# zoongahn/jodalroB-twoTower

Hardware: AMD Instinct MI355X
Metric: training pairs/sec at batch 8192 (embedding-lookup HBM GB/s in roofline) (higher is better)
Workload: dtype bf16 MFMA operands, f32 accumulate; f32 tables, master weights and activations (the tower input x, which the GEMMs round to bf16 anyway, is stored bf16)

## Files before the change

### jodalrob-twotower_amd/csrc/tt_gemm.h

```cpp
#pragma once
#include "tt_common.h"

struct GemmNT {
  const float* A; int64_t lda; const float* W; int64_t ldw; const float* bias; float* C; int64_t ldc;
  int64_t M, N, K; bool relu; float alpha; bool bf16 = false;
  void* workspace = nullptr; size_t workspace_bytes = 0;
  bool a_bf16 = false, c_bf16 = false;
  struct NtDeferred* defer = nullptr;
};
struct NtDeferred { const float* slabs; int64_t slab_stride; int splits; };
size_t tt_gemm_nt_workspace_bytes(int64_t M, int64_t N, int64_t K);
int tt_gemm_nt_batched(hipStream_t st, const GemmNT* items, int n);
int tt_gemm_nt(hipStream_t st, const float* A, int64_t lda, const float* W, int64_t ldw, const float* bias, float* C,
               int64_t ldc, int64_t M, int64_t N, int64_t K, bool relu, float alpha = 1.f);

struct GemmNN {
  const float* A; int64_t lda; const float* W; int64_t ldw; float* C; int64_t ldc; int64_t M, N, K; bool bf16 = false;
  bool c_bf16 = false;
};
int tt_gemm_nn_batched(hipStream_t st, const GemmNN* items, int n);

size_t tt_gemm_tn_workspace_bytes(int64_t M, int64_t N, int64_t R);
struct GemmTN {
  const float* A; int64_t lda; const float* B; int64_t ldb; float* C; int64_t ldc; int64_t M, N, R;
// ... 108 lines not shown

struct GemmBack {
  const float* dpre; int H;
  const void* x; int64_t ldx; int kx; bool x_bf16;
  const float* dense; int64_t ld_dense; int din;
  const float* w; int h0;
  float* dx; int64_t ld_dx; bool dx_bf16;
  float* dw; float* db; float* dwp; float* dbp;
  void* ws_dw; size_t ws_dw_bytes;
  void* ws_g; size_t ws_g_bytes;
  int64_t B;
  const void* w16 = nullptr;
};
bool tt_gemm_back_supported(const GemmBack* items, int n);
size_t tt_gemm_back_g_workspace_bytes(int64_t H, int64_t h0, int64_t din, int64_t B);
int tt_gemm_back_batched(hipStream_t st, const GemmBack* items, int n, TnPending* pending);
```

### jodalrob-twotower_amd/csrc/tt_gemm.hip

```cpp
#include "tt_gemm.h"

#include <stdlib.h>

namespace {

constexpr int BM = 64, BN = 64, BK = 16, PAD = 4, THREADS = 256;
using f32x16 = __attribute__((ext_vector_type(16))) float;

struct GemmArgs {
  const float* A; int64_t lda; const float* B; int64_t ldb; float* C; int64_t ldc; int64_t slab_stride;
  int M, N, K, kchunk, splits;
  const float* bias; int relu; float alpha; float* colsum_slab;
  int a_bf16 = 0, b_bf16 = 0, c_bf16 = 0;
  const float* proj_w = nullptr; int proj_ldw = 0, proj_h0 = 0;
};
struct GemmBatch { GemmArgs a[TT_MAX_SIDES]; };

template <int MODE, bool VEC>
struct TileLoader {
  float r[4];
  __device__ __forceinline__ void load(const float* __restrict__ P, int64_t ld, int x0, int X, int k0, int kend, int t) {
    if (MODE == 0) {
      const int row = t >> 2, kq = (t & 3) * 4;
      const int x = x0 + row, k = k0 + kq;
// ... 495 lines not shown
      const int m = m0 + wr * 32 + (r & 3) + 8 * (r >> 2) + 4 * lh;
      if (g.c_bf16) reinterpret_cast<uint16_t*>(g.C)[(int64_t)m * g.ldc + n] = tt_f2bf(acc[r]);
      else g.C[(int64_t)m * g.ldc + n] = acc[r];
    }
    __syncthreads();
  }
}

constexpr int kBackProbs = 3 * TT_MAX_SIDES;
struct BackBatch {
  GemmArgs g[kBackProbs];
  int role[kBackProbs], tiles_m[kBackProbs], tiles[kBackProbs], wg_end[kBackProbs];
  int n;
};

template <bool X_BF16>
__global__ __launch_bounds__(THREADS, 4) void gemm_back_kernel(BackBatch b) {
  int p = 0;
  while (p + 1 < b.n && (int)blockIdx.x >= b.wg_end[p]) ++p;
  const int local = (int)blockIdx.x - (p ? b.wg_end[p - 1] : 0);
  const int split = local / b.tiles[p], tile = local % b.tiles[p];
  const int bx = tile % b.tiles_m[p], by = tile / b.tiles_m[p];
  __shared__ __attribute__((aligned(16))) BackSmem sm;
  const GemmArgs& g = b.g[p];
  if (b.role[p] == 0) gemm_fast_tile<1, 1, true, false, X_BF16>(g, split, bx, by, sm);
  else if (b.role[p] == 1) gemm_fast_tile<1, 1, false, false, false, true>(g, split, bx, by, sm);
  else if (g.K == 64) {
    const int nt_cols = g.N / BN;
    if (g.b_bf16) gemm_nn_k64_tiles<true>(g, bx, by * kNnCols, min(kNnCols, nt_cols - by * kNnCols), sm);
    else gemm_nn_k64_tiles<false>(g, bx, by * kNnCols, min(kNnCols, nt_cols - by * kNnCols), sm);
  } else gemm_fast_tile<0, 1, false, false, false>(g, split, bx, by, sm);
}

__global__ __launch_bounds__(THREADS) void slab_reduce_kernel(SlabBatch batch) {
  slab_reduce_block(batch, (int)blockIdx.x, (int)gridDim.x, (int)blockIdx.y);
}

inline bool vec_ok(const float* p, int64_t ld, bool bf16_elems = false) {
// ... 232 lines not shown
  for (int i = 0; i < n; ++i) {
    const GemmBack& g = it[i];
    if (g.B < 64 || g.B % 64 || g.H < 64 || g.H % 64 || g.H > kProjMaxH || g.kx % 64 || g.h0 % 64 || g.h0 < 64 || g.h0 >= g.kx || g.din % 64) return false;
    if ((g.H / BM) * g.h0 > 256) return false;
    if (g.x_bf16 != it[0].x_bf16) return false;
    if (!tt_aligned(g.dpre, 16) || !tt_aligned(g.x, 16) || g.ldx % 8 || !tt_aligned(g.dense, 16) || g.ld_dense % 4 || !tt_aligned(g.w, 16) ||
        !tt_aligned(g.dx, 16) || g.ld_dx % 4)
      return false;
    if (!g.ws_dw || g.ws_dw_bytes < tt_gemm_tn_workspace_bytes(g.H, g.kx, g.B) || !g.ws_g ||
        g.ws_g_bytes < tt_gemm_back_g_workspace_bytes(g.H, g.h0, g.din, g.B))
      return false;
  }
  return true;
}

int tt_gemm_back_batched(hipStream_t st, const GemmBack* it, int n, TnPending* pending) {
  if (!pending || !tt_gemm_back_supported(it, n)) {
    tt_set_error("tt_gemm_back: unsupported shapes / missing pending queue");
    return TT_ERR_INVALID_ARG;
  }
  BackBatch b{};
  SlabArgs sa[3 * TT_MAX_SIDES];
  int ns = 0, wg = 0;
  int64_t maxtotal = 1;
  auto kchunk_of = [](int64_t R, int splits) { return (int)(tt_cdiv(tt_cdiv(R, splits), BK16) * BK16); };
  for (int role = 0; role < 3; ++role)
    for (int i = 0; i < n; ++i) {
      const GemmBack& g = it[i];
      const int s0 = tn_splits(g.H, g.kx, g.B), s1 = back_g_splits(g.H, g.din, g.B);
      float* slabs0 = reinterpret_cast<float*>((reinterpret_cast<uintptr_t>(g.ws_dw) + 255) & ~uintptr_t(255));
      float* cslab0 = slabs0 + (size_t)s0 * (size_t)g.H * (size_t)g.kx;
// ... 19 lines not shown
      } else {
        float* c = g.dx_bf16 ? reinterpret_cast<float*>(reinterpret_cast<uint16_t*>(g.dx) + g.h0) : g.dx + g.h0;
        const bool w16 = g.w16 != nullptr && g.H == 64 && tt_aligned(g.w16, 16);
        const float* wsrc = w16 ? reinterpret_cast<const float*>(reinterpret_cast<const uint16_t*>(g.w16) + g.h0) : g.w + g.h0;
        b.g[p] = GemmArgs{g.dpre, g.H, wsrc, g.kx, c, g.ld_dx, 0, (int)g.B, g.kx - g.h0, g.H, (int)(tt_cdiv(g.H, BK16) * BK16), 1,
                          nullptr, 0, 1.f, nullptr, 0, w16 ? 1 : 0, g.dx_bf16 ? 1 : 0};
        tm = (int)(g.B / BM); tn_ = (g.kx - g.h0) / BN;
        if (g.H == 64) tn_ = (int)tt_cdiv(tn_, kNnCols);
      }
      b.role[p] = role;
      b.tiles_m[p] = tm;
      b.tiles[p] = tm * tn_;
      wg += tm * tn_ * b.g[p].splits;
      b.wg_end[p] = wg;
    }
  if (it[0].x_bf16) gemm_back_kernel<true><<<wg, THREADS, 0, st>>>(b);
  else gemm_back_kernel<false><<<wg, THREADS, 0, st>>>(b);
  TT_LAUNCH_CHECK();
  if (pending->n + ns > kSlabItems)
    if (int rc = tt_gemm_tn_flush(st, pending)) return rc;
  for (int i = 0; i < ns; ++i) pending->sb.a[pending->n++] = sa[i];
  pending->maxtotal = maxtotal > pending->maxtotal ? maxtotal : pending->maxtotal;
  return TT_OK;
}

int tt_gemm_nt(hipStream_t st, const float* A, int64_t lda, const float* W, int64_t ldw, const float* bias, float* C,
               int64_t ldc, int64_t M, int64_t N, int64_t K, bool relu, float alpha) {
  GemmNT it{A, lda, W, ldw, bias, C, ldc, M, N, K, relu, alpha};
  return tt_gemm_nt_batched(st, &it, 1);
}
```

### jodalrob-twotower_amd/csrc/tt_riders.h

```cpp
#pragma once
#include "tt_common.h"

constexpr int kRiderThreads = 1024;
constexpr int kPlanLongSeg = 64;
struct PlanLong {
  int32_t* counters;
  int32_t* long_row; int32_t* long_base; int32_t* chunk_lo; int32_t* chunk_hi;
};
struct CompactRider {
  const int32_t* uniq_stage; const int32_t* seg_stage; const int32_t* ucount; const int32_t* ubase; const int32_t* uend;
  PlanLong pl;
  int n_keys; int64_t M;
  int32_t* unique_rows; int32_t* seg_offsets; int32_t* n_unique;
};
struct Finish2Rider {
  const float* part; int n_wg, Dp; float fb, unscale; float* out; float* loss_out;
};
struct BnFinishRider {
  const float* partial; int64_t pstride; int nchunks, H;
  float* mean; float* rstd; float* rm; float* rv; int64_t* nbt;
  float* out;
};
struct BnFinishRiders { BnFinishRider r[TT_MAX_SIDES]; };
constexpr int kBnFinStride = 2 * 64;
// ... 144 lines not shown
        pl.long_row[li] = before + u;
        pl.long_base[li] = cb;
        for (int32_t c = 0; c < nch; ++c) {
          pl.chunk_lo[cb + c] = s0 + c * kPlanLongSeg;
          pl.chunk_hi[cb + c] = min(s1, s0 + (c + 1) * kPlanLongSeg);
        }
      }
    }
  }
  if (ki == 0 && threadIdx.x == 0) {
    n_unique[0] = all;
    seg_offsets[all] = (int32_t)M;
  }
}

__device__ __forceinline__ void finish2_body(const Finish2Rider& fr) {
  const float* __restrict__ part = fr.part;
  const int n_wg = fr.n_wg, Dp = fr.Dp;
  const float fb = fr.fb, unscale = fr.unscale;
  float* __restrict__ out = fr.out;
  float* __restrict__ loss_out = fr.loss_out;

  __shared__ float red[4][4 + 2 * 256];
  __shared__ float prod[256];
  const int t = threadIdx.x, q = t >> 8, j0 = t & 255, stride = 4 + 2 * Dp;
  for (int j = j0; j < stride; j += 256) {
    float s = 0.f;
    for (int w0 = q; w0 < n_wg; w0 += 32) {
      float v[8];
#pragma unroll
      for (int k = 0; k < 8; ++k) v[k] = w0 + 4 * k < n_wg ? part[(int64_t)(w0 + 4 * k) * stride + j] : 0.f;
#pragma unroll
      for (int k = 0; k < 8; ++k) s += v[k];
    }
    red[q][j] = s;
  }
  __syncthreads();
  if (t < 256) {
    float p = 0.f;
    if (t < Dp) {
      const float u = (red[0][4 + t] + red[1][4 + t]) + (red[2][4 + t] + red[3][4 + t]);
      const float v = (red[0][4 + Dp + t] + red[1][4 + Dp + t]) + (red[2][4 + Dp + t] + red[3][4 + Dp + t]);
      p = u * v;
    }
    prod[t] = p;
  }
  __syncthreads();
  if (t < 64) {
    float p = (prod[t] + prod[t + 64]) + (prod[t + 128] + prod[t + 192]);
#pragma unroll
// ... 5 lines not shown
      const float dsum = (red[0][2] + red[1][2]) + (red[2][2] + red[3][2]);
      const float pos = dsum / fb;
      const float neg = (tot - dsum) / (fb * fb - fb);
      out[0] = 0.5f * l / fb;
      out[1] = hit / fb;
      out[2] = pos;
      out[3] = neg;
      out[4] = pos - neg;
      out[5] = 0.f;
      out[6] = tot;
      out[7] = 0.f;
      if (loss_out) loss_out[0] = out[0];
    }
  }
}
#endif
```

### jodalrob-twotower_amd/csrc/tt_score_bf16.hip

```cpp
#include "tt_score_bwd_parts.h"
#include "tt_tail_bwd.h"
#include "tt_deferred.h"

#include <stdlib.h>

namespace {

template <int KS, int AT>
__device__ __forceinline__ void mfma1(const bf16x8 (&bf)[KS], const bf16x8 (&ares)[AT][KS], f32x16 (&acc)[AT]) {
#pragma unroll
  for (int i = 0; i < AT; ++i)
#pragma unroll
    for (int r = 0; r < 16; ++r) acc[i][r] = 0.f;
#pragma unroll
  for (int s = 0; s < KS; ++s)
#pragma unroll
    for (int i = 0; i < AT; ++i) acc[i] = __builtin_amdgcn_mfma_f32_32x32x16_bf16(bf[s], ares[i][s], acc[i], 0, 0, 0);
}

template <int KS, int AT, bool X3>
__device__ __forceinline__ void mfma_s(const bf16x8 (&bh)[KS], const bf16x8 (&bl)[X3 ? KS : 1], const bf16x8 (&ah)[AT][KS],
                                       const bf16x8 (&al)[AT][X3 ? KS : 1], f32x16 (&acc)[AT]) {
  if constexpr (!X3) {
    mfma1<KS, AT>(bh, ah, acc);
// ... 448 lines not shown
          if (a < Ra && dd < args.D) dr.dA[(int64_t)a * args.D + dd] = dacc[i][d][r] * g;
        }
  }
}

template <bool TAIL>
struct TailHost {};
template <>
struct TailHost<true> { tttail::Batch<tttail::TailBwdArgs> batch; bool drop; float p; uint64_t seed0; const uint64_t* seed_dev; };

template <int KS, int AT, bool UNIT, bool LQ = false, bool TAIL = false>
__global__ __launch_bounds__(512) void score_bwd_tr_kernel(BwdArgs args, TailHost<TAIL> th) {
  constexpr int NW = 8, Dp = KS * 16, ROWS = 32 * AT, DT = KS / 2;
  constexpr int TLD = Dp + 8;
  constexpr int kRedB = (NW / 2) * ROWS * Dp * 4, kParkB = NW * 32 * TLD * 2;
  static_assert(!TAIL || (KS == 4 && AT == 2 && !LQ && tttail::kTailBwdLds + 64 * tttail::kTailTileLd * 4 <= kRedB + kParkB),
                "the tail's head and its d_emb tile lie over red | park of the <4, 2> form");
  __shared__ float red_s[TAIL ? 1 : (NW / 2) * ROWS * Dp];
  __shared__ __attribute__((aligned(16))) __bf16 park_s[TAIL ? 1 : NW][32 * TLD];
  __shared__ __attribute__((aligned(16))) char smem[TAIL ? kRedB + kParkB : 16];
  float* const red = TAIL ? reinterpret_cast<float*>(smem) : red_s;
  __bf16 (*const park)[32 * TLD] = TAIL ? reinterpret_cast<__bf16 (*)[32 * TLD]>(smem + kRedB) : park_s;
  using s16x4 = __attribute__((ext_vector_type(4))) short;
  using s16x8 = __attribute__((ext_vector_type(8))) short;
  const BwdSel dr = select_dir(args, blockIdx.y != 0);
  const float c1 = dr.c1, c2 = args.c2, kx = UNIT ? args.kexp : 1.f;
  const int Ra = dr.Ra, Rb = dr.Rb, off = dr.off;
  const float* const wt_b = dr.wt_b;
  const int a0 = (int)blockIdx.x * ROWS;
  if (a0 >= Ra) return;
  const int lane = threadIdx.x & 63, c = lane & 31, h = lane >> 5;
  const int wave = __builtin_amdgcn_readfirstlane(threadIdx.x >> 6);
  const int nT = (Rb + 31) / 32;
  bf16x8 ares[AT][KS];
  float ia[AT], ua[AT];
  int pos[AT];
#pragma unroll
  for (int i = 0; i < AT; ++i) {
    load_bfrag<KS>(dr.a_rows, a0 / 32 + i, c, h, ares[i]);
    a_row_setup<LQ>(dr, kx, a0 + 32 * i + c, ia[i], ua[i], pos[i]);
  }
  const int posmin = a0 + off, posmax = a0 + ROWS - 1 + off;
  f32x16 dacc[AT][DT];
  zero_acc(dacc);
  const bool have_inv = dr.inv_b != nullptr;
// ... 85 lines not shown
    }
  };
  Tile T0, T1;
  load(T0, min(wave, tlast));
  __builtin_amdgcn_sched_barrier(0);
  for (int t = wave; t < nT; t += 2 * NW) {
    load(T1, min(t + NW, tlast));
    compute(T0, t);
    load(T0, min(t + 2 * NW, tlast));
    if (t + NW < nT) compute(T1, t + NW);
  }
  [[maybe_unused]] tttail::TailBwdConst<512> hk;
  [[maybe_unused]] tttail::TailBwdRows<512> hv;
  [[maybe_unused]] uint64_t hseed = 0;
  if constexpr (TAIL) {
    const tttail::TailBwdArgs& f = th.batch.a[blockIdx.y];
    tttail::tail_bwd_load_const<512>(f, hk);
    tttail::tail_bwd_load_rows<512, true>(f, min(f.col.B, a0 + 64), a0, hv);
    if (th.drop) hseed = tttail::seed_of(th.seed0, th.seed_dev);
  }
#pragma unroll
  for (int half = NW / 2; half >= 1; half >>= 1) {
    if (wave >= half && wave < 2 * half) {
      float* slab = red + (wave - half) * ROWS * Dp;
#pragma unroll
      for (int i = 0; i < AT; ++i)
#pragma unroll
        for (int d = 0; d < DT; ++d)
#pragma unroll
          for (int r = 0; r < 16; ++r) slab[(32 * i + rowmap(r, h)) * Dp + 32 * d + c] = dacc[i][d][r];
    }
    __syncthreads();
    if (wave < half) {
      const float* slab = red + wave * ROWS * Dp;
#pragma unroll
      for (int i = 0; i < AT; ++i)
#pragma unroll
        for (int d = 0; d < DT; ++d)
#pragma unroll
          for (int r = 0; r < 16; ++r) dacc[i][d][r] += slab[(32 * i + rowmap(r, h)) * Dp + 32 * d + c];
    }
    __syncthreads();
  }
  [[maybe_unused]] float* const htile = reinterpret_cast<float*>(smem + tttail::kTailBwdLds);
  if (wave == 0) {
    const float g = args.d_loss[0] * dr.out_scale;
#pragma unroll
    for (int i = 0; i < AT; ++i)
#pragma unroll
      for (int d = 0; d < DT; ++d)
#pragma unroll
        for (int r = 0; r < 16; ++r) {
          const int a = a0 + 32 * i + rowmap(r, h);
          const int dd = 32 * d + c;
          if (a < Ra && dd < args.D) dr.dA[(int64_t)a * args.D + dd] = dacc[i][d][r] * g;
          if constexpr (TAIL) htile[(32 * i + rowmap(r, h)) * tttail::kTailTileLd + dd] = dacc[i][d][r] * g;
        }
  }
  if constexpr (TAIL) tttail::tail_bwd_head<512, true>(th.batch.a[blockIdx.y], blockIdx.x, th.drop, th.p, hseed, smem, htile, &hk, &hv);
}

template <int KS, bool UNIT, bool FP8, int AT, int NWV, bool LQ = false>
__global__ __launch_bounds__(NWV * 64) void score_bwd_rows_kernel(BwdArgs args) {
  constexpr int NTH = NWV * 64, DT = KS / 2, Dp = KS * 16, K64 = FP8 ? KS / 4 : 1;
  constexpr int kRowsB = FP8 ? KS * 512 : KS * 1024, kFragB = KS * 1024, kIvB = 256, kStageB = kRowsB + kFragB + kIvB;
  constexpr int kPieces = (kRowsB + kFragB) / 16, kPPT = (kPieces + NTH - 1) / NTH;
  static_assert(!FP8 || KS % 4 == 0, "fp8 operands come in K = 64 steps");
  constexpr bool ALDS = !FP8 && KS == 16;
  extern __shared__ __attribute__((aligned(16))) char lds_raw[];
  const bool d1 = blockIdx.y != 0;
  DirBwd dr;
  dr.a_rows = d1 ? args.d[1].a_rows : args.d[0].a_rows;
  dr.b_rows = d1 ? args.d[1].b_rows : args.d[0].b_rows;
  dr.b_frag = d1 ? args.d[1].b_frag : args.d[0].b_frag;
// ... 655 lines not shown
                        tt_stream stream) {
  return fwd_bf16(ctx, dirs, n_dirs, D, inv_t, shift, stream, true, "tt_score_fwd_bf16x3");
}

int tt_score_bwd_bf16x3(tt_ctx* ctx, const tt_score_bwd_dir* dirs, int32_t n_dirs, int32_t D, float inv_t, float shift,
                        const float* d_loss, float scale, tt_stream stream) {
  return bwd_bf16x3(ctx, dirs, nullptr, n_dirs, D, inv_t, shift, d_loss, scale, stream, "tt_score_bwd_bf16x3");
}

int tt_score_bwd_bf16x3_lq(tt_ctx* ctx, const tt_score_bwd_dir* dirs, const tt_score_bwd_lq* lq, int32_t n_dirs, int32_t D,
                           float inv_t, float shift, const float* d_loss, float scale, tt_stream stream) {
  TT_CHECK_ARG(lq, "tt_score_bwd_bf16x3_lq: NULL lq");
  return bwd_bf16x3(ctx, dirs, lq, n_dirs, D, inv_t, shift, d_loss, scale, stream, "tt_score_bwd_bf16x3_lq");
}

}
```

### jodalrob-twotower_amd/csrc/tt_tail_bwd.h

```cpp
#pragma once
#include "tt_common.h"

namespace tttail {

constexpr float kNormEps = 1e-12f;

__device__ __forceinline__ float dropout_scale(bool on, float p, uint64_t seed, uint64_t idx) {
  if (!on) return 1.f;
  return tt_uniform01(seed, idx) >= p ? 1.f / (1.f - p) : 0.f;
}
__device__ __forceinline__ uint64_t seed_of(uint64_t seed, const uint64_t* seed_dev) { return seed_dev ? seed + seed_dev[0] : seed; }

template <typename A>
struct Batch {
  A a[TT_MAX_SIDES];
};

struct ColArgs {
  const float* x; int64_t ldx;
  const float* pre; const float* mean; const float* rstd;
  uint64_t salt;
  int B, H, rows_per_chunk, nchunks;
  float* partial; float* out0; float* out1;
  int64_t pstride = 0;
// ... 8 lines not shown

using tl_f32x16 = __attribute__((ext_vector_type(16))) float;
using tl_bf16x8 = __attribute__((ext_vector_type(8))) __bf16;
constexpr int kTailLd = 72;
constexpr int kTailLdF = 65;

struct TailBwdArgs {
  const float* y; const float* emb; const float* d_emb; float* d_y; int D;
  const float* w_out; const float* act; float* d_act;
  ColArgs col;
  float* w_slab; float* b_slab;
};

constexpr int kTailBwdLds = 2 * (2 * 64 * kTailLd) + 2 * (64 * kTailLd) + 2 * (64 * kTailLd) + 4 * (64 * kTailLdF) + 4 * (3 * 4 * 64);
static_assert(sizeof(float) * 64 * kTailLdF <= sizeof(__bf16) * 2 * 64 * kTailLd, "XH must fit over dyA | dyT");
constexpr int kTailTileLd = 72;

template <int NT>
struct TailBwdConst {
  static constexpr int R = 64 * 64 / NT;
  float w[R], mean, rstd;
};
template <int NT>
struct TailBwdRows {
  static constexpr int R = 64 * 64 / NT;
  float yv[R], e[R], de[R], av[R], pr[R];
};

template <int NT>
__device__ __forceinline__ void tail_bwd_load_const(const TailBwdArgs& f, TailBwdConst<NT>& k) {
  constexpr int NWV = NT / 64, R = TailBwdConst<NT>::R;
  const int H = f.col.H, D = f.D;
  const int c = threadIdx.x & 63, rq = threadIdx.x >> 6;
#pragma unroll
  for (int j = 0; j < R; ++j) {
    const int d = rq + NWV * j;
    k.w[j] = f.w_out[(int64_t)min(d, D - 1) * H + min(c, H - 1)];
  }
  k.mean = c < H ? f.col.mean[c] : 0.f;
  k.rstd = c < H ? f.col.rstd[c] : 0.f;
}

template <int NT, bool TILE>
__device__ __forceinline__ void tail_bwd_load_rows(const TailBwdArgs& f, int r1, int b0, TailBwdRows<NT>& v) {
  constexpr int NWV = NT / 64, R = TailBwdRows<NT>::R;
  const int H = f.col.H, D = f.D;
  const int c = threadIdx.x & 63, rq = threadIdx.x >> 6;
  const int lane = c, wave = rq;
#pragma unroll
  for (int j = 0; j < R; ++j) {
    const int r = b0 + wave * R + j;
    const bool ok = r < r1 && lane < D;
    const int64_t i = (int64_t)min(r, r1 - 1) * D + min(lane, D - 1);
    const float v0 = f.y[i], v1 = f.emb[i];
    v.yv[j] = ok ? v0 : 0.f;
    v.e[j] = ok ? v1 : 0.f;
    if constexpr (!TILE) {
      const float v2 = f.d_emb[i];
      v.de[j] = ok ? v2 : 0.f;
    }
  }
#pragma unroll
  for (int j = 0; j < R; ++j) {
    const int r = b0 + rq + NWV * j;
    const bool ok = c < H && r < r1;
    const int64_t i = (int64_t)min(r, r1 - 1) * H + min(c, H - 1);
    const float v0 = f.act[i], v1 = f.col.pre[i];
    v.av[j] = ok ? v0 : 0.f;
    v.pr[j] = ok ? v1 : 0.f;
  }
}

template <int NT, bool TILE>
__device__ __forceinline__ void tail_bwd_head(const TailBwdArgs& f, int chunk, bool drop, float p, uint64_t seed, char* smem,
                                              const float* tile, const TailBwdConst<NT>* pk, const TailBwdRows<NT>* pv) {
  static_assert(NT == 1024 || NT == 512, "the ordered parts run in the first four waves; the rest splits 64 rows over NT / 64");
  constexpr int NWV = NT / 64, R = 64 * 64 / NT;
  const ColArgs& a = f.col;
  const int H = a.H, D = f.D;
  __bf16* dy2 = reinterpret_cast<__bf16*>(smem);
  __bf16* Wn = dy2 + 2 * 64 * kTailLd;
  __bf16* actT = Wn + 64 * kTailLd;
  float* DY = reinterpret_cast<float*>(actT + 64 * kTailLd);
  float (*sh)[4][64] = reinterpret_cast<float (*)[4][64]>(DY + 64 * kTailLdF);
  __bf16* dyA = dy2;
  __bf16* dyT = dy2 + 64 * kTailLd;
  float* XH = reinterpret_cast<float*>(dy2);
  const int t = threadIdx.x, c = t & 63, rq = t >> 6;
  const int lane = c, wave = rq;
  const int r0 = chunk * a.rows_per_chunk, r1 = min(a.B, r0 + a.rows_per_chunk);
  TailBwdConst<NT> k;
  if constexpr (TILE) k = *pk;
  else tail_bwd_load_const<NT>(f, k);
#pragma unroll
  for (int j = 0; j < R; ++j) {
    const int d = rq + NWV * j;
    Wn[c * kTailLd + d] = (__bf16)((d < D && c < H) ? k.w[j] : 0.f);
  }
  const float mean = k.mean, rstd = k.rstd;
  tl_f32x16 accw;
#pragma unroll
  for (int i = 0; i < 16; ++i) accw[i] = 0.f;
  float s0 = 0.f, s1 = 0.f, cs = 0.f;
  for (int b0 = r0; b0 < r1; b0 += 64) {
    TailBwdRows<NT> v;
    if constexpr (TILE) {
      v = *pv;
      __syncthreads();
#pragma unroll
      for (int j = 0; j < R; ++j) {
        const int row = wave * R + j;
        const float v2 = tile[row * kTailTileLd + lane];
        v.de[j] = (b0 + row < r1 && lane < D) ? v2 : 0.f;
      }
    } else {
      tail_bwd_load_rows<NT, false>(f, r1, b0, v);
    }
    float ss[R], dot[R], xh[R], sc[R];
#pragma unroll
    for (int j = 0; j < R; ++j) {
      ss[j] = mul_rn(v.yv[j], v.yv[j]);
      dot[j] = mul_rn(v.e[j], v.de[j]);
    }
#pragma unroll
    for (int o = 32; o > 0; o >>= 1) {
#pragma unroll
      for (int j = 0; j < R; ++j) {
        ss[j] += __shfl_xor(ss[j], o);
        dot[j] += __shfl_xor(dot[j], o);
// ... 7 lines not shown
      float out = nrm > kNormEps ? (v.de[j] - v.e[j] * dot[j]) / den : v.de[j] / den;
      if (r < r1 && lane < D) f.d_y[(int64_t)r * D + lane] = out;
      else out = 0.f;
      DY[row * kTailLdF + lane] = out;
      dyA[row * kTailLd + lane] = (__bf16)out;
      dyT[lane * kTailLd + row] = (__bf16)out;
    }
#pragma unroll
    for (int j = 0; j < R; ++j) {
      const int row = rq + NWV * j, r = b0 + row;
      actT[c * kTailLd + row] = (__bf16)v.av[j];
      xh[j] = (fmaxf(v.pr[j], 0.f) - mean) * rstd;
      sc[j] = (c < H && r < r1) ? dropout_scale(drop, p, seed, a.salt + (uint64_t)((int64_t)r * H + c)) : 0.f;
    }
    __syncthreads();
    const int wr = (wave >> 1) & 1, wc = wave & 1, li = lane & 31, lh = lane >> 5;
    tl_f32x16 acc;
#pragma unroll
    for (int i = 0; i < 16; ++i) acc[i] = 0.f;
    if (wave < 4) {
      if (c < D) {
#pragma unroll
        for (int j = 0; j < 16; ++j) cs += DY[(rq + 4 * j) * kTailLdF + c];
      }
#pragma unroll
      for (int s2 = 0; s2 < 4; ++s2) {
        const int ko = 16 * s2 + 8 * lh;
        const tl_bf16x8 a1 = *reinterpret_cast<const tl_bf16x8*>(dyA + (wr * 32 + li) * kTailLd + ko);
        const tl_bf16x8 b1 = *reinterpret_cast<const tl_bf16x8*>(Wn + (wc * 32 + li) * kTailLd + ko);
        acc = __builtin_amdgcn_mfma_f32_32x32x16_bf16(a1, b1, acc, 0, 0, 0);
        const tl_bf16x8 a2 = *reinterpret_cast<const tl_bf16x8*>(dyT + (wr * 32 + li) * kTailLd + ko);
        const tl_bf16x8 b2 = *reinterpret_cast<const tl_bf16x8*>(actT + (wc * 32 + li) * kTailLd + ko);
        accw = __builtin_amdgcn_mfma_f32_32x32x16_bf16(a2, b2, accw, 0, 0, 0);
      }
    }
    __syncthreads();
    if (wave < 4) {
      const int n = wc * 32 + li;
#pragma unroll
      for (int r = 0; r < 16; ++r) DY[(wr * 32 + (r & 3) + 8 * (r >> 2) + 4 * lh) * kTailLdF + n] = acc[r];
    }
    __syncthreads();
#pragma unroll
    for (int j = 0; j < R; ++j) {
      const int row = rq + NWV * j, r = b0 + row;
      const float da = DY[row * kTailLdF + c] * sc[j];
      if (c < H && r < r1) f.d_act[(int64_t)r * H + c] = da;
      DY[row * kTailLdF + c] = da;
      XH[row * kTailLdF + c] = xh[j];
    }
    __syncthreads();
    if (t < 256 && c < H) {
      const int nrow = min(64, r1 - b0);
      for (int row = rq; row < nrow; row += 4) {
        const float da = DY[row * kTailLdF + c];
        s0 += da;
        s1 += da * XH[row * kTailLdF + c];
      }
    }
    __syncthreads();
  }
  if (t < 256) {
    sh[0][rq][c] = s0;
    sh[1][rq][c] = s1;
    sh[2][rq][c] = cs;
  }
  __syncthreads();
  if (t < 64) {
    if (c < H) {
      float* q = a.partial + (int64_t)chunk * 2 * H;
      q[c] = ((sh[0][0][c] + sh[0][1][c]) + sh[0][2][c]) + sh[0][3][c];
      q[H + c] = ((sh[1][0][c] + sh[1][1][c]) + sh[1][2][c]) + sh[1][3][c];
    }
    if (c < D) f.b_slab[(int64_t)chunk * D + c] = ((sh[2][0][c] + sh[2][1][c]) + sh[2][2][c]) + sh[2][3][c];
  }
  if (wave < 4) {
    const int wr = wave >> 1, wc = wave & 1, li = lane & 31, lh = lane >> 5;
    float* ws = f.w_slab + (int64_t)chunk * D * H;
    const int n = wc * 32 + li;
#pragma unroll
    for (int r = 0; r < 16; ++r) {
      const int m = wr * 32 + (r & 3) + 8 * (r >> 2) + 4 * lh;
      if (m < D && n < H) ws[(int64_t)m * H + n] = accw[r];
    }
  }
}

}

int tt_score_tail_bwd_launch(tt_ctx* ctx, const tttail::Batch<tttail::TailBwdArgs>& tb, bool drop, float p, uint64_t seed,
                             const uint64_t* seed_dev);
```

### jodalrob-twotower_amd/csrc/tt_tower.hip

```cpp
#include "tt_deferred.h"
#include "tt_tail_bwd.h"

namespace {

using namespace tttail;

constexpr int kThreads = 256;

struct BnStatArgs {
  const float* pre; int B, H, rows_per_chunk, nchunks; float* partial; float* mean; float* rstd; float* rm; float* rv; int64_t* nbt;
  int64_t pstride = 0;
};

__global__ __launch_bounds__(kThreads) void bn_stats_partial_kernel(Batch<BnStatArgs> batch) {
  const BnStatArgs& a = batch.a[blockIdx.z];
  const int H = a.H;
  if ((int)blockIdx.x * 64 >= H || (int)blockIdx.y >= a.nchunks) return;
  __shared__ Wf sh[4][64];
  const int c = blockIdx.x * 64 + (threadIdx.x & 63), rl = threadIdx.x >> 6;
  const int r0 = blockIdx.y * a.rows_per_chunk, r1 = min(a.B, r0 + a.rows_per_chunk);
  Wf w{0.f, 0.f, 0.f};
  if (c < H && r0 + rl < r1) {
    const float x0 = fmaxf(a.pre[(int64_t)(r0 + rl) * H + c], 0.f);
    float s = 0.f, q = 0.f, cnt = 0.f;
// ... 914 lines not shown
      *reinterpret_cast<bf16x4*>(f.pk_frag + fi * 8 + (q >> 3) * 4) = o;
    }
  }
}

__global__ __launch_bounds__(kTailThreads) void tail_bwd_kernel(Batch<TailBwdArgs> batch, bool drop, float p, uint64_t seed0,
                                                               const uint64_t* __restrict__ seed_dev, Finish2Rider fr, int fr_on) {
  if (fr_on && blockIdx.y == 0) {
    if (blockIdx.x == 0) finish2_body(fr);
    return;
  }
  const TailBwdArgs& f = batch.a[blockIdx.y - fr_on];
  if ((int)blockIdx.x >= f.col.nchunks) return;
  __shared__ __attribute__((aligned(16))) char smem[kTailBwdLds];
  const uint64_t seed = drop ? seed_of(seed0, seed_dev) : 0;
  tail_bwd_head<kTailThreads, false>(f, blockIdx.x, drop, p, seed, smem, nullptr, nullptr, nullptr);
}

struct TailApplyArgs {
  ColArgs col; BnBwdArgs bn;
  const float* w_slab; const float* b_slab; int D; float* g_w_out; float* g_b_out;
  int slab_chunks;
  float out_scale;
};

__global__ __launch_bounds__(kTailThreads) void tail_bwd_apply_kernel(Batch<TailApplyArgs> batch, Finish2Rider fr, int fr_on) {
  if (fr_on && blockIdx.y == 0) {
    if (blockIdx.x == 0) finish2_body(fr);
    return;
  }
  const TailApplyArgs& ta = batch.a[blockIdx.y - fr_on];
// ... 714 lines not shown
    TT_LAUNCH_CHECK();
  }
  for (int t = 0; t < n; ++t) {
    const tt_tower_grads* g = G[t];
    const float* in_last = nh == 0 ? reinterpret_cast<const float*>(A[t]->x) : A[t]->act[nh - 1];
    const int lw = last_width(P[t]);
    tn[t] = GemmTN{g->d_y, P[t]->d_out, in_last, lw, g->w_out, lw, P[t]->d_out, lw, B, ws[t].tn[nh + 1], ws[t].tn_bytes[nh + 1], g->b_out};
    dcur[t] = nh == 0 ? reinterpret_cast<float*>(g->d_x) : g->scratch[nh - 1];
    TT_CHECK_ARG(dcur[t], "tt_towers_mlp_bwd: NULL scratch buffer");
    nn[t] = GemmNN{g->d_y, P[t]->d_out, P[t]->w_out, lw, dcur[t], lw, B, lw, P[t]->d_out};
    tn[t].b_bf16 = nh == 0 && P[t]->x_dtype == TT_BF16;
    nn[t].c_bf16 = nh == 0 && P[t]->dx_dtype == TT_BF16;
  }
  for (int t = 0; t < n; ++t) tn[t].bf16 = nn[t].bf16 = P[0]->compute_dtype == TT_BF16;
  TnPending pend;
  if (fused) {
    const int i = nh - 1;
    Batch<TailBwdArgs> tb{};
    Batch<TailApplyArgs> tp{};
    int cmax = 1;
    for (int t = 0; t < n; ++t) {
      const tt_tower_grads* g = G[t];
      const int H = P[t]->hidden[i], D = P[t]->d_out;
      TT_CHECK_ARG(g->w[i] && g->b[i] && g->bn_w[i] && g->bn_b[i], "tt_towers_mlp_bwd: NULL gradient buffers of block %d", i);
      const int nchunks = chunks_for(B, H);
      const uint64_t salt = (((uint64_t)(i + 1) << 40) ^ ((uint64_t)t << 52)) + (uint64_t)P[t]->rng_row_offset * (uint64_t)H;
      const ColArgs col{nullptr, 0, A[t]->pre[i], A[t]->mean[i], A[t]->rstd[i], salt, (int)B, H, (int)tt_cdiv(B, nchunks), nchunks,
                        ws[t].col, g->bn_b[i], g->bn_w[i]};
      float* w_slab = reinterpret_cast<float*>((reinterpret_cast<uintptr_t>(ws[t].tn[nh + 1]) + 255) & ~uintptr_t(255));
      float* b_slab = w_slab + (size_t)nchunks * D * H;
// ... 22 lines not shown
    const int fr_on = (mine & TT_DQ_LOSS) ? 1 : 0;
    if (phase != 2 && !hosted) {
      tail_bwd_kernel<<<dim3((unsigned)cmax, (unsigned)(n + fr_on)), kTailThreads, 0, st>>>(tb, drop, dropout_p, seed, seed_dev, ctx->dq->loss,
                                                                                           fr_on);
      tt_deferred_taken(ctx, TT_DQ_LOSS & mine);
      TT_LAUNCH_CHECK();
    }
    if (phase == 1) {
      Batch<LocalArgs> la{};
      for (int t = 0; t < n; ++t) la.a[t] = LocalArgs{tb.a[t].col.partial, tb.a[t].col.nchunks, tb.a[t].col.H, G[t]->s_sync_local};
      tail_local_colsum_kernel<<<dim3(1, (unsigned)n), kThreads, 0, st>>>(la);
      TT_LAUNCH_CHECK();
      return TT_OK;
    }
    {
      const int fr_here = hosted ? fr_on : 0;
      tail_bwd_apply_kernel<<<dim3((unsigned)tt_cdiv(B, 64), (unsigned)(n + fr_here)), kTailThreads, 0, st>>>(tp, ctx->dq->loss, fr_here);
      if (fr_here) tt_deferred_taken(ctx, TT_DQ_LOSS);
      TT_LAUNCH_CHECK();
    }
  } else if (wide) {
    const int i = nh - 1;
    if (phase != 2) {
      Batch<TailBwdArgs> tb{};
      int cmax = 1;
      for (int t = 0; t < n; ++t) {
        const int H = P[t]->hidden[i];
        const int nchunks = chunks_for(B, H);
        const uint64_t salt = (((uint64_t)(i + 1) << 40) ^ ((uint64_t)t << 52)) + (uint64_t)P[t]->rng_row_offset * (uint64_t)H;
        const ColArgs col{nullptr, 0, A[t]->pre[i], A[t]->mean[i], A[t]->rstd[i], salt, (int)B, H, (int)tt_cdiv(B, nchunks), nchunks,
                          ws[t].col, G[t]->bn_b[i], G[t]->bn_w[i]};
// ... 68 lines not shown
    for (int t = 0; t < n; ++t) {
      const tt_tower_grads* g = G[t];
      const int H = P[t]->hidden[i];
      const int iw = in_width(P[t], i);
      const float* in_i = i == 0 ? reinterpret_cast<const float*>(A[t]->x) : A[t]->act[i - 1];
      tn[t] = GemmTN{dcur[t], H, in_i, iw, g->w[i], iw, H, iw, B, ws[t].tn[1 + i], ws[t].tn_bytes[1 + i], g->b[i]};
      tn[t].b_bf16 = i == 0 && P[t]->x_dtype == TT_BF16;
      float* dnext = i == 0 ? reinterpret_cast<float*>(g->d_x) : g->scratch[i - 1];
      TT_CHECK_ARG(dnext, "tt_towers_mlp_bwd: NULL scratch buffer");
      nn[t] = GemmNN{dcur[t], H, P[t]->w[i], iw, dnext, iw, B, iw, H};
      nn[t].c_bf16 = i == 0 && P[t]->dx_dtype == TT_BF16;
      dcur[t] = dnext;
    }
    for (int t = 0; t < n; ++t) tn[t].bf16 = nn[t].bf16 = P[0]->compute_dtype == TT_BF16;
    if (i == 0 && P[0]->compute_dtype == TT_BF16) {
      GemmBack gb[TT_MAX_SIDES];
      bool ok = true;
      for (int t = 0; t < n; ++t) {
        const tt_tower_grads* g = G[t];
        const int wx = P[t]->h0 + P[t]->kcat_e;
        ok = ok && !(P[t]->flags & TT_TOWER_UNFUSED_BACK);
        gb[t] = GemmBack{tn[t].A, P[t]->hidden[0], A[t]->x, wx, wx, P[t]->x_dtype == TT_BF16, A[t]->dense, P[t]->din, P[t]->din,
                         P[t]->w[0], P[t]->h0, reinterpret_cast<float*>(g->d_x), wx, P[t]->dx_dtype == TT_BF16, g->w[0], g->b[0],
                         g->w_proj, g->b_proj, ws[t].tn[1], ws[t].tn_bytes[1], ws[t].tn[0], ws[t].tn_bytes[0], B};
        gb[t].w16 = P[t]->w_bf16[0];
      }
      if (ok && tt_gemm_back_supported(gb, n)) {
        if (int rc = tt_gemm_back_batched(st, gb, n, &pend)) return rc;
        if (ctx->dq->defer_slabs) return tt_deferred_queue_slabs(ctx, st, &pend);
        return tt_gemm_tn_flush(st, &pend);
      }
    }
    if (int rc = tt_gemm_tn_batched(st, tn, n, &pend)) return rc;
    if (int rc = tt_gemm_nn_batched(st, nn, n)) return rc;
  }
  for (int t = 0; t < n; ++t) {
    const tt_tower_grads* g = G[t];
    const int wx = P[t]->h0 + P[t]->kcat_e;
    tn[t] = GemmTN{reinterpret_cast<const float*>(g->d_x), wx, A[t]->dense, P[t]->din, g->w_proj, P[t]->din, P[t]->h0, P[t]->din, B,
                   ws[t].tn[0], ws[t].tn_bytes[0], g->b_proj};
    tn[t].a_bf16 = P[t]->dx_dtype == TT_BF16;
  }
  for (int t = 0; t < n; ++t) tn[t].bf16 = P[0]->compute_dtype == TT_BF16;
// ... 32 lines not shown
```

Before: 37.33 million.

## Move loss-finish rider into gemm_back and keep tail d_emb in registers

The deferred loss reduction (finish2) now rides as an extra workgroup of the fused backward GEMM kernel instead of the tail-apply kernel, reusing the GEMM's LDS. In the fused score-backward tail, the wave reduction is restructured into a single-level split-and-sum in which each thread reads its rows of d_emb straight into registers. This replaces the staged LDS tile and the extra sync inside tail_bwd_head. Optional timestamp probes are added behind a compile flag. This is meant to shorten the tail-apply critical path and cut LDS traffic, at the cost of more register pressure and a heavier first GEMM block.

```diff
diff --git a/jodalrob-twotower_amd/csrc/tt_gemm.h b/jodalrob-twotower_amd/csrc/tt_gemm.h
--- a/jodalrob-twotower_amd/csrc/tt_gemm.h
+++ b/jodalrob-twotower_amd/csrc/tt_gemm.h
@@ -1,5 +1,6 @@
 #pragma once
 #include "tt_common.h"
+#include "tt_riders.h"
 
 struct GemmNT {
   const float* A; int64_t lda; const float* W; int64_t ldw; const float* bias; float* C; int64_t ldc;
@@ -146,4 +147,4 @@
 };
 bool tt_gemm_back_supported(const GemmBack* items, int n);
 size_t tt_gemm_back_g_workspace_bytes(int64_t H, int64_t h0, int64_t din, int64_t B);
-int tt_gemm_back_batched(hipStream_t st, const GemmBack* items, int n, TnPending* pending);
+int tt_gemm_back_batched(hipStream_t st, const GemmBack* items, int n, TnPending* pending, const Finish2Rider* rider = nullptr);
diff --git a/jodalrob-twotower_amd/csrc/tt_gemm.hip b/jodalrob-twotower_amd/csrc/tt_gemm.hip
--- a/jodalrob-twotower_amd/csrc/tt_gemm.hip
+++ b/jodalrob-twotower_amd/csrc/tt_gemm.hip
@@ -533,14 +533,20 @@
   int n;
 };
 
+static_assert(sizeof(BackSmem) >= sizeof(float) * kFinish2Lds, "the loss reduction runs in the tiles' LDS");
 template <bool X_BF16>
-__global__ __launch_bounds__(THREADS, 4) void gemm_back_kernel(BackBatch b) {
+__global__ __launch_bounds__(THREADS, 4) void gemm_back_kernel(BackBatch b, Finish2Rider fr, int fr_on) {
+  __shared__ __attribute__((aligned(16))) BackSmem sm;
+  if (fr_on && blockIdx.x == 0) {
+    finish2_body<THREADS>(fr, reinterpret_cast<float*>(&sm));
+    return;
+  }
+  const int wg = (int)blockIdx.x - fr_on;
   int p = 0;
-  while (p + 1 < b.n && (int)blockIdx.x >= b.wg_end[p]) ++p;
-  const int local = (int)blockIdx.x - (p ? b.wg_end[p - 1] : 0);
+  while (p + 1 < b.n && wg >= b.wg_end[p]) ++p;
+  const int local = wg - (p ? b.wg_end[p - 1] : 0);
   const int split = local / b.tiles[p], tile = local % b.tiles[p];
   const int bx = tile % b.tiles_m[p], by = tile / b.tiles_m[p];
-  __shared__ __attribute__((aligned(16))) BackSmem sm;
   const GemmArgs& g = b.g[p];
   if (b.role[p] == 0) gemm_fast_tile<1, 1, true, false, X_BF16>(g, split, bx, by, sm);
   else if (b.role[p] == 1) gemm_fast_tile<1, 1, false, false, false, true>(g, split, bx, by, sm);
@@ -803,7 +809,7 @@
   return true;
 }
 
-int tt_gemm_back_batched(hipStream_t st, const GemmBack* it, int n, TnPending* pending) {
+int tt_gemm_back_batched(hipStream_t st, const GemmBack* it, int n, TnPending* pending, const Finish2Rider* rider) {
   if (!pending || !tt_gemm_back_supported(it, n)) {
     tt_set_error("tt_gemm_back: unsupported shapes / missing pending queue");
     return TT_ERR_INVALID_ARG;
@@ -853,8 +859,10 @@
       wg += tm * tn_ * b.g[p].splits;
       b.wg_end[p] = wg;
     }
-  if (it[0].x_bf16) gemm_back_kernel<true><<<wg, THREADS, 0, st>>>(b);
-  else gemm_back_kernel<false><<<wg, THREADS, 0, st>>>(b);
+  const int fr_on = rider ? 1 : 0;
+  const Finish2Rider fr = rider ? *rider : Finish2Rider{};
+  if (it[0].x_bf16) gemm_back_kernel<true><<<wg + fr_on, THREADS, 0, st>>>(b, fr, fr_on);
+  else gemm_back_kernel<false><<<wg + fr_on, THREADS, 0, st>>>(b, fr, fr_on);
   TT_LAUNCH_CHECK();
   if (pending->n + ns > kSlabItems)
     if (int rc = tt_gemm_tn_flush(st, pending)) return rc;
diff --git a/jodalrob-twotower_amd/csrc/tt_riders.h b/jodalrob-twotower_amd/csrc/tt_riders.h
--- a/jodalrob-twotower_amd/csrc/tt_riders.h
+++ b/jodalrob-twotower_amd/csrc/tt_riders.h
@@ -182,26 +182,40 @@
   }
 }
 
-__device__ __forceinline__ void finish2_body(const Finish2Rider& fr) {
+constexpr int kFinish2Lds = 4 * (4 + 2 * 256) + 256;
+template <int NT>
+__device__ __forceinline__ void finish2_body(const Finish2Rider& fr, float* lds) {
+  static_assert(NT >= 256 && kRiderThreads % NT == 0, "thread t stands in for the threads t + NT i of a kRiderThreads workgroup");
+  constexpr int NI = kRiderThreads / NT;
   const float* __restrict__ part = fr.part;
   const int n_wg = fr.n_wg, Dp = fr.Dp;
   const float fb = fr.fb, unscale = fr.unscale;
   float* __restrict__ out = fr.out;
   float* __restrict__ loss_out = fr.loss_out;
 
-  __shared__ float red[4][4 + 2 * 256];
-  __shared__ float prod[256];
-  const int t = threadIdx.x, q = t >> 8, j0 = t & 255, stride = 4 + 2 * Dp;
+  float (*red)[4 + 2 * 256] = reinterpret_cast<float (*)[4 + 2 * 256]>(lds);
+  float* prod = lds + 4 * (4 + 2 * 256);
+  const int t = threadIdx.x, q0 = t >> 8, j0 = t & 255, stride = 4 + 2 * Dp;
   for (int j = j0; j < stride; j += 256) {
-    float s = 0.f;
-    for (int w0 = q; w0 < n_wg; w0 += 32) {
-      float v[8];
-#pragma unroll
-      for (int k = 0; k < 8; ++k) v[k] = w0 + 4 * k < n_wg ? part[(int64_t)(w0 + 4 * k) * stride + j] : 0.f;
-#pragma unroll
-      for (int k = 0; k < 8; ++k) s += v[k];
-    }
-    red[q][j] = s;
+    float s[NI];
+#pragma unroll
+    for (int i = 0; i < NI; ++i) s[i] = 0.f;
+    for (int w0 = q0; w0 < n_wg; w0 += 32) {
+      float v[NI][8];
+#pragma unroll
+      for (int i = 0; i < NI; ++i)
+#pragma unroll
+        for (int k = 0; k < 8; ++k) {
+          const int w = w0 + (NT / 256) * i + 4 * k;
+          v[i][k] = w < n_wg ? part[w * stride + j] : 0.f;
+        }
+#pragma unroll
+      for (int i = 0; i < NI; ++i)
+#pragma unroll
+        for (int k = 0; k < 8; ++k) s[i] += v[i][k];
+    }
+#pragma unroll
+    for (int i = 0; i < NI; ++i) red[q0 + (NT / 256) * i][j] = s[i];
   }
   __syncthreads();
   if (t < 256) {
@@ -237,4 +251,8 @@
     }
   }
 }
+__device__ __forceinline__ void finish2_body(const Finish2Rider& fr) {
+  __shared__ float lds[kFinish2Lds];
+  finish2_body<kRiderThreads>(fr, lds);
+}
 #endif
diff --git a/jodalrob-twotower_amd/csrc/tt_score_bf16.hip b/jodalrob-twotower_amd/csrc/tt_score_bf16.hip
--- a/jodalrob-twotower_amd/csrc/tt_score_bf16.hip
+++ b/jodalrob-twotower_amd/csrc/tt_score_bf16.hip
@@ -1,4 +1,11 @@
 #include "tt_score_bwd_parts.h"
+#ifdef TT_POST_STAMPS
+__device__ unsigned long long g_post_stamps[512 * 16];
+#define TT_POST_STAMP(i) do { if (threadIdx.x == 0) g_post_stamps[((blockIdx.y * gridDim.x + blockIdx.x) & 511) * 16 + (i)] = __builtin_amdgcn_s_memrealtime(); } while (0)
+#define TT_HEAD_STAMP(i) TT_POST_STAMP(8 + (i))
+#else
+#define TT_POST_STAMP(i) do { } while (0)
+#endif
 #include "tt_tail_bwd.h"
 #include "tt_deferred.h"
 
@@ -486,8 +493,8 @@
   constexpr int NW = 8, Dp = KS * 16, ROWS = 32 * AT, DT = KS / 2;
   constexpr int TLD = Dp + 8;
   constexpr int kRedB = (NW / 2) * ROWS * Dp * 4, kParkB = NW * 32 * TLD * 2;
-  static_assert(!TAIL || (KS == 4 && AT == 2 && !LQ && tttail::kTailBwdLds + 64 * tttail::kTailTileLd * 4 <= kRedB + kParkB),
-                "the tail's head and its d_emb tile lie over red | park of the <4, 2> form");
+  static_assert(!TAIL || (KS == 4 && AT == 2 && !LQ && tttail::kTailBwdLds <= kRedB + kParkB),
+                "the tail's head lies over red | park of the <4, 2> form");
   __shared__ float red_s[TAIL ? 1 : (NW / 2) * ROWS * Dp];
   __shared__ __attribute__((aligned(16))) __bf16 park_s[TAIL ? 1 : NW][32 * TLD];
   __shared__ __attribute__((aligned(16))) char smem[TAIL ? kRedB + kParkB : 16];
@@ -501,6 +508,7 @@
   const float* const wt_b = dr.wt_b;
   const int a0 = (int)blockIdx.x * ROWS;
   if (a0 >= Ra) return;
+  if constexpr (TAIL) TT_POST_STAMP(0);
   const int lane = threadIdx.x & 63, c = lane & 31, h = lane >> 5;
   const int wave = __builtin_amdgcn_readfirstlane(threadIdx.x >> 6);
   const int nT = (Rb + 31) / 32;
@@ -616,15 +624,16 @@
   [[maybe_unused]] tttail::TailBwdRows<512> hv;
   [[maybe_unused]] uint64_t hseed = 0;
   if constexpr (TAIL) {
+    TT_POST_STAMP(1);
     const tttail::TailBwdArgs& f = th.batch.a[blockIdx.y];
     tttail::tail_bwd_load_const<512>(f, hk);
     tttail::tail_bwd_load_rows<512, true>(f, min(f.col.B, a0 + 64), a0, hv);
     if (th.drop) hseed = tttail::seed_of(th.seed0, th.seed_dev);
-  }
-#pragma unroll
-  for (int half = NW / 2; half >= 1; half >>= 1) {
-    if (wave >= half && wave < 2 * half) {
-      float* slab = red + (wave - half) * ROWS * Dp;
+    TT_POST_STAMP(2);
+  }
+  if constexpr (TAIL) {
+    if (wave >= NW / 2) {
+      float* slab = red + (wave - NW / 2) * ROWS * Dp;
 #pragma unroll
       for (int i = 0; i < AT; ++i)
 #pragma unroll
@@ -633,33 +642,76 @@
           for (int r = 0; r < 16; ++r) slab[(32 * i + rowmap(r, h)) * Dp + 32 * d + c] = dacc[i][d][r];
     }
     __syncthreads();
-    if (wave < half) {
-      const float* slab = red + wave * ROWS * Dp;
+    TT_POST_STAMP(3);
+    if (wave < NW / 2) {
+      float* slab = red + wave * ROWS * Dp;
 #pragma unroll
       for (int i = 0; i < AT; ++i)
 #pragma unroll
         for (int d = 0; d < DT; ++d)
 #pragma unroll
-          for (int r = 0; r < 16; ++r) dacc[i][d][r] += slab[(32 * i + rowmap(r, h)) * Dp + 32 * d + c];
+          for (int r = 0; r < 16; ++r) {
+            float* at = slab + (32 * i + rowmap(r, h)) * Dp + 32 * d + c;
+            *at = dacc[i][d][r] + *at;
+          }
     }
     __syncthreads();
-  }
-  [[maybe_unused]] float* const htile = reinterpret_cast<float*>(smem + tttail::kTailBwdLds);
-  if (wave == 0) {
+    TT_POST_STAMP(4);
+    const tttail::TailBwdArgs& f = th.batch.a[blockIdx.y];
     const float g = args.d_loss[0] * dr.out_scale;
-#pragma unroll
-    for (int i = 0; i < AT; ++i)
-#pragma unroll
-      for (int d = 0; d < DT; ++d)
-#pragma unroll
-        for (int r = 0; r < 16; ++r) {
-          const int a = a0 + 32 * i + rowmap(r, h);
-          const int dd = 32 * d + c;
-          if (a < Ra && dd < args.D) dr.dA[(int64_t)a * args.D + dd] = dacc[i][d][r] * g;
-          if constexpr (TAIL) htile[(32 * i + rowmap(r, h)) * tttail::kTailTileLd + dd] = dacc[i][d][r] * g;
-        }
-  }
-  if constexpr (TAIL) tttail::tail_bwd_head<512, true>(th.batch.a[blockIdx.y], blockIdx.x, th.drop, th.p, hseed, smem, htile, &hk, &hv);
+    constexpr int R = tttail::TailBwdRows<512>::R;
+    static_assert(R * NW == ROWS && Dp == 64, "thread (wave, lane): rows wave R .. wave R + R - 1 of column lane");
+#pragma unroll
+    for (int j = 0; j < R; ++j) {
+      const float* at = red + (wave * R + j) * Dp + lane;
+      const float s0 = at[0], s1 = at[ROWS * Dp], s2 = at[2 * ROWS * Dp], s3 = at[3 * ROWS * Dp];
+      const float v = ((s0 + s2) + (s1 + s3)) * g;
+      const int a = a0 + wave * R + j;
+      if (a < Ra && lane < args.D) dr.dA[(int64_t)a * args.D + lane] = v;
+      hv.de[j] = (a < f.col.B && lane < f.D) ? v : 0.f;
+    }
+    TT_POST_STAMP(5);
+    __syncthreads();
+    TT_POST_STAMP(6);
+    tttail::tail_bwd_head<512, true>(f, blockIdx.x, th.drop, th.p, hseed, smem, &hk, &hv);
+  } else {
+#pragma unroll
+    for (int half = NW / 2; half >= 1; half >>= 1) {
+      if (wave >= half && wave < 2 * half) {
+        float* slab = red + (wave - half) * ROWS * Dp;
+#pragma unroll
+        for (int i = 0; i < AT; ++i)
+#pragma unroll
+          for (int d = 0; d < DT; ++d)
+#pragma unroll
+            for (int r = 0; r < 16; ++r) slab[(32 * i + rowmap(r, h)) * Dp + 32 * d + c] = dacc[i][d][r];
+      }
+      __syncthreads();
+      if (wave < half) {
+        const float* slab = red + wave * ROWS * Dp;
+#pragma unroll
+        for (int i = 0; i < AT; ++i)
+#pragma unroll
+          for (int d = 0; d < DT; ++d)
+#pragma unroll
+            for (int r = 0; r < 16; ++r) dacc[i][d][r] += slab[(32 * i + rowmap(r, h)) * Dp + 32 * d + c];
+      }
+      __syncthreads();
+    }
+    if (wave == 0) {
+      const float g = args.d_loss[0] * dr.out_scale;
+#pragma unroll
+      for (int i = 0; i < AT; ++i)
+#pragma unroll
+        for (int d = 0; d < DT; ++d)
+#pragma unroll
+          for (int r = 0; r < 16; ++r) {
+            const int a = a0 + 32 * i + rowmap(r, h);
+            const int dd = 32 * d + c;
+            if (a < Ra && dd < args.D) dr.dA[(int64_t)a * args.D + dd] = dacc[i][d][r] * g;
+          }
+    }
+  }
 }
 
 template <int KS, bool UNIT, bool FP8, int AT, int NWV, bool LQ = false>
@@ -1345,4 +1397,10 @@
   return bwd_bf16x3(ctx, dirs, lq, n_dirs, D, inv_t, shift, d_loss, scale, stream, "tt_score_bwd_bf16x3_lq");
 }
 
-}
+#ifdef TT_POST_STAMPS
+int tt_debug_post_stamps(unsigned long long* host_out ) {
+  return hipMemcpyFromSymbol(host_out, HIP_SYMBOL(g_post_stamps), sizeof(unsigned long long) * 512 * 16, 0, hipMemcpyDeviceToHost) == hipSuccess ? 0 : -2;
+}
+#endif
+
+}
diff --git a/jodalrob-twotower_amd/csrc/tt_tail_bwd.h b/jodalrob-twotower_amd/csrc/tt_tail_bwd.h
--- a/jodalrob-twotower_amd/csrc/tt_tail_bwd.h
+++ b/jodalrob-twotower_amd/csrc/tt_tail_bwd.h
@@ -1,5 +1,9 @@
 #pragma once
 #include "tt_common.h"
+
+#ifndef TT_HEAD_STAMP
+#define TT_HEAD_STAMP(i) do { } while (0)
+#endif
 
 namespace tttail {
 
@@ -46,7 +50,6 @@
 
 constexpr int kTailBwdLds = 2 * (2 * 64 * kTailLd) + 2 * (64 * kTailLd) + 2 * (64 * kTailLd) + 4 * (64 * kTailLdF) + 4 * (3 * 4 * 64);
 static_assert(sizeof(float) * 64 * kTailLdF <= sizeof(__bf16) * 2 * 64 * kTailLd, "XH must fit over dyA | dyT");
-constexpr int kTailTileLd = 72;
 
 template <int NT>
 struct TailBwdConst {
@@ -73,7 +76,7 @@
   k.rstd = c < H ? f.col.rstd[c] : 0.f;
 }
 
-template <int NT, bool TILE>
+template <int NT, bool REGS>
 __device__ __forceinline__ void tail_bwd_load_rows(const TailBwdArgs& f, int r1, int b0, TailBwdRows<NT>& v) {
   constexpr int NWV = NT / 64, R = TailBwdRows<NT>::R;
   const int H = f.col.H, D = f.D;
@@ -87,7 +90,7 @@
     const float v0 = f.y[i], v1 = f.emb[i];
     v.yv[j] = ok ? v0 : 0.f;
     v.e[j] = ok ? v1 : 0.f;
-    if constexpr (!TILE) {
+    if constexpr (!REGS) {
       const float v2 = f.d_emb[i];
       v.de[j] = ok ? v2 : 0.f;
     }
@@ -103,9 +106,9 @@
   }
 }
 
-template <int NT, bool TILE>
+template <int NT, bool REGS>
 __device__ __forceinline__ void tail_bwd_head(const TailBwdArgs& f, int chunk, bool drop, float p, uint64_t seed, char* smem,
-                                              const float* tile, const TailBwdConst<NT>* pk, const TailBwdRows<NT>* pv) {
+                                              const TailBwdConst<NT>* pk, const TailBwdRows<NT>* pv) {
   static_assert(NT == 1024 || NT == 512, "the ordered parts run in the first four waves; the rest splits 64 rows over NT / 64");
   constexpr int NWV = NT / 64, R = 64 * 64 / NT;
   const ColArgs& a = f.col;
@@ -122,7 +125,7 @@
   const int lane = c, wave = rq;
   const int r0 = chunk * a.rows_per_chunk, r1 = min(a.B, r0 + a.rows_per_chunk);
   TailBwdConst<NT> k;
-  if constexpr (TILE) k = *pk;
+  if constexpr (REGS) k = *pk;
   else tail_bwd_load_const<NT>(f, k);
 #pragma unroll
   for (int j = 0; j < R; ++j) {
@@ -136,15 +139,8 @@
   float s0 = 0.f, s1 = 0.f, cs = 0.f;
   for (int b0 = r0; b0 < r1; b0 += 64) {
     TailBwdRows<NT> v;
-    if constexpr (TILE) {
+    if constexpr (REGS) {
       v = *pv;
-      __syncthreads();
-#pragma unroll
-      for (int j = 0; j < R; ++j) {
-        const int row = wave * R + j;
-        const float v2 = tile[row * kTailTileLd + lane];
-        v.de[j] = (b0 + row < r1 && lane < D) ? v2 : 0.f;
-      }
     } else {
       tail_bwd_load_rows<NT, false>(f, r1, b0, v);
     }
@@ -182,6 +178,7 @@
       sc[j] = (c < H && r < r1) ? dropout_scale(drop, p, seed, a.salt + (uint64_t)((int64_t)r * H + c)) : 0.f;
     }
     __syncthreads();
+    TT_HEAD_STAMP(0);
     const int wr = (wave >> 1) & 1, wc = wave & 1, li = lane & 31, lh = lane >> 5;
     tl_f32x16 acc;
 #pragma unroll
@@ -203,12 +200,14 @@
       }
     }
     __syncthreads();
+    TT_HEAD_STAMP(1);
     if (wave < 4) {
       const int n = wc * 32 + li;
 #pragma unroll
       for (int r = 0; r < 16; ++r) DY[(wr * 32 + (r & 3) + 8 * (r >> 2) + 4 * lh) * kTailLdF + n] = acc[r];
     }
     __syncthreads();
+    TT_HEAD_STAMP(2);
 #pragma unroll
     for (int j = 0; j < R; ++j) {
       const int row = rq + NWV * j, r = b0 + row;
@@ -218,6 +217,7 @@
       XH[row * kTailLdF + c] = xh[j];
     }
     __syncthreads();
+    TT_HEAD_STAMP(3);
     if (t < 256 && c < H) {
       const int nrow = min(64, r1 - b0);
       for (int row = rq; row < nrow; row += 4) {
@@ -227,6 +227,7 @@
       }
     }
     __syncthreads();
+    TT_HEAD_STAMP(4);
   }
   if (t < 256) {
     sh[0][rq][c] = s0;
@@ -234,6 +235,7 @@
     sh[2][rq][c] = cs;
   }
   __syncthreads();
+  TT_HEAD_STAMP(5);
   if (t < 64) {
     if (c < H) {
       float* q = a.partial + (int64_t)chunk * 2 * H;
@@ -252,6 +254,7 @@
       if (m < D && n < H) ws[(int64_t)m * H + n] = accw[r];
     }
   }
+  TT_HEAD_STAMP(6);
 }
 
 }
diff --git a/jodalrob-twotower_amd/csrc/tt_tower.hip b/jodalrob-twotower_amd/csrc/tt_tower.hip
--- a/jodalrob-twotower_amd/csrc/tt_tower.hip
+++ b/jodalrob-twotower_amd/csrc/tt_tower.hip
@@ -952,7 +952,7 @@
   if ((int)blockIdx.x >= f.col.nchunks) return;
   __shared__ __attribute__((aligned(16))) char smem[kTailBwdLds];
   const uint64_t seed = drop ? seed_of(seed0, seed_dev) : 0;
-  tail_bwd_head<kTailThreads, false>(f, blockIdx.x, drop, p, seed, smem, nullptr, nullptr, nullptr);
+  tail_bwd_head<kTailThreads, false>(f, blockIdx.x, drop, p, seed, smem, nullptr, nullptr);
 }
 
 struct TailApplyArgs {
@@ -1697,6 +1697,21 @@
   }
   for (int t = 0; t < n; ++t) tn[t].bf16 = nn[t].bf16 = P[0]->compute_dtype == TT_BF16;
   TnPending pend;
+  GemmBack gb[TT_MAX_SIDES];
+  auto back_items = [&]() {
+    if (nh < 1 || P[0]->compute_dtype != TT_BF16) return false;
+    for (int t = 0; t < n; ++t) {
+      const tt_tower_grads* g = G[t];
+      const int wx = P[t]->h0 + P[t]->kcat_e;
+      if (P[t]->flags & TT_TOWER_UNFUSED_BACK) return false;
+      gb[t] = GemmBack{g->scratch[0], P[t]->hidden[0], A[t]->x, wx, wx, P[t]->x_dtype == TT_BF16, A[t]->dense, P[t]->din, P[t]->din,
+                       P[t]->w[0], P[t]->h0, reinterpret_cast<float*>(g->d_x), wx, P[t]->dx_dtype == TT_BF16, g->w[0], g->b[0],
+                       g->w_proj, g->b_proj, ws[t].tn[1], ws[t].tn_bytes[1], ws[t].tn[0], ws[t].tn_bytes[0], B};
+      gb[t].w16 = P[t]->w_bf16[0];
+    }
+    return tt_gemm_back_supported(gb, n);
+  };
+  bool loss_to_back = false;
   if (fused) {
     const int i = nh - 1;
     Batch<TailBwdArgs> tb{};
@@ -1749,7 +1764,8 @@
       return TT_OK;
     }
     {
-      const int fr_here = hosted ? fr_on : 0;
+      loss_to_back = hosted && fr_on && back_items();
+      const int fr_here = hosted && fr_on && !loss_to_back ? 1 : 0;
       tail_bwd_apply_kernel<<<dim3((unsigned)tt_cdiv(B, 64), (unsigned)(n + fr_here)), kTailThreads, 0, st>>>(tp, ctx->dq->loss, fr_here);
       if (fr_here) tt_deferred_taken(ctx, TT_DQ_LOSS);
       TT_LAUNCH_CHECK();
@@ -1848,19 +1864,12 @@
     }
     for (int t = 0; t < n; ++t) tn[t].bf16 = nn[t].bf16 = P[0]->compute_dtype == TT_BF16;
     if (i == 0 && P[0]->compute_dtype == TT_BF16) {
-      GemmBack gb[TT_MAX_SIDES];
-      bool ok = true;
-      for (int t = 0; t < n; ++t) {
-        const tt_tower_grads* g = G[t];
-        const int wx = P[t]->h0 + P[t]->kcat_e;
-        ok = ok && !(P[t]->flags & TT_TOWER_UNFUSED_BACK);
-        gb[t] = GemmBack{tn[t].A, P[t]->hidden[0], A[t]->x, wx, wx, P[t]->x_dtype == TT_BF16, A[t]->dense, P[t]->din, P[t]->din,
-                         P[t]->w[0], P[t]->h0, reinterpret_cast<float*>(g->d_x), wx, P[t]->dx_dtype == TT_BF16, g->w[0], g->b[0],
-                         g->w_proj, g->b_proj, ws[t].tn[1], ws[t].tn_bytes[1], ws[t].tn[0], ws[t].tn_bytes[0], B};
-        gb[t].w16 = P[t]->w_bf16[0];
-      }
-      if (ok && tt_gemm_back_supported(gb, n)) {
-        if (int rc = tt_gemm_back_batched(st, gb, n, &pend)) return rc;
+      if (back_items()) {
+        int mine = 0;
+        if (loss_to_back)
+          if (int rc = tt_deferred_host(ctx, TT_DQ_LOSS, st, &mine)) return rc;
+        if (int rc = tt_gemm_back_batched(st, gb, n, &pend, (mine & TT_DQ_LOSS) ? &ctx->dq->loss : nullptr)) return rc;
+        tt_deferred_taken(ctx, mine & TT_DQ_LOSS);
         if (ctx->dq->defer_slabs) return tt_deferred_queue_slabs(ctx, st, &pend);
         return tt_gemm_tn_flush(st, &pend);
       }
```

Result: faster. 38.20 million, median of 6 (+2.3%).
